# bikuta6/nbody-deep-sim

Hardware: AMD Instinct MI355X
Metric: pair-interactions/sec, direct O(N^2) leapfrog N-body, fp32 (higher is better)
Workload: dtype f32; 1 GPU; Plummer sphere, 65536 particles, direct all-pairs leapfrog step (BASELINE configs[1] shape: 65536 bodies per GPU); n_particles=65536, particles_per_gpu=65536, seed=1234, parallelism=single GPU

## Files before the change

### include/nbd.h

```cpp
#ifndef NBD_H_
#define NBD_H_

#include <stddef.h>
#include <stdint.h>

#ifdef __cplusplus
extern "C" {
#endif

#define NBD_ABI_VERSION 2
#define NBD_E_BADARG (-1)
#define NBD_E_WORKSPACE (-2)
#define NBD_E_UNSUPPORTED (-3)

#define NBD_SRC_PAD 64
#define NBD_CC_TILE 128
#define NBD_CC_GROUPS 8
#define NBD_CC_MAX_RES 4

typedef void* nbd_stream_t;

int nbd_abi_version(void);
size_t nbd_struct_size(const char* name);
const char* nbd_strerror(int code);
// ... 10 lines not shown
int nbd_accel_f32(const float* posm_src, int n_src, const float* posm_tgt, int n_tgt,
                  int tgt_global_offset, float softening_sq, float g_const, float* acc_out,
                  void* workspace, size_t workspace_bytes, nbd_stream_t stream);

size_t nbd_accel_tuned_workspace_bytes(int n_tgt, int slabs);
int nbd_accel_tuned_f32(const float* posm_src, int n_src, int exclude_lo, int exclude_hi, const float* posm_tgt,
                        int n_tgt, int tgt_global_offset, float softening_sq, float g_const, float* acc_out,
                        void* workspace, size_t workspace_bytes, int slabs, int variant, nbd_stream_t stream);

int nbd_shard_plan(int n_total, int lo, int n_local, int* slabs_local, int* chunks_per_wave_local,
                   int* slabs_remote, int* chunks_per_wave_remote);
size_t nbd_shard_workspace_bytes(int n_total, int lo, int n_local);
int nbd_shard_force_local_f32(const float* posm_local, int n_local, float softening_sq, void* workspace,
                              size_t workspace_bytes, int n_total, int lo, nbd_stream_t stream);
int nbd_shard_force_remote_f32(const float* posm_all, int n_total, const float* posm_local, int n_local, int lo,
                               float softening_sq, float g_const, float* acc_out, float* vel, float c_kick,
                               void* workspace, size_t workspace_bytes, nbd_stream_t stream);
int nbd_shard_force_local_uniform_f32(const float* posm_local, int n_local, float softening_sq, void* workspace,
                                      size_t workspace_bytes, int n_total, int lo, nbd_stream_t stream);
int nbd_shard_force_remote_uniform_f32(const float* posm_all, int n_total, const float* posm_local, int n_local, int lo,
                                       float softening_sq, float g_const, float mass_value, float* acc_out, float* vel,
                                       float c_kick, void* workspace, size_t workspace_bytes, nbd_stream_t stream);

int nbd_kick_drift_f32(float* pos, float* vel, const float* acc, const float* mass, int n,
                       float c_kick, float c_drift, float* posm, nbd_stream_t stream);

int nbd_kick_f32(float* vel, const float* acc, int n, float c, nbd_stream_t stream);

int nbd_drift_f32(float* pos, const float* vel, int n, float c, nbd_stream_t stream);

int nbd_snapshot_f32(const float* pos, const float* vel, const float* acc, int n, float* out, nbd_stream_t stream);

size_t nbd_step_workspace_bytes(int n);

size_t nbd_step_workspace_pref_bytes(int n);

int nbd_leapfrog_step_f32(float* pos, float* vel, const float* acc_in, float* acc_out,
                          const float* mass, int n, float dt_half, float dt, float softening_sq,
                          float g_const, float* posm, void* workspace, size_t workspace_bytes,
                          nbd_stream_t stream);

int nbd_leapfrog_step_ev_f32(float* pos, float* vel, const float* acc_in, float* acc_out,
                             const float* mass, int n, float dt_half, float dt, float softening_sq,
                             float g_const, float* posm, void* workspace, size_t workspace_bytes,
                             nbd_stream_t stream, void* ev_force_begin, void* ev_force_end);
int nbd_leapfrog_step_uniform_f32(float* pos, float* vel, const float* acc_in, float* acc_out, const float* mass,
                                  float mass_value, int n, float dt_half, float dt, float softening_sq, float g_const,
                                  float* posm, void* workspace, size_t workspace_bytes, nbd_stream_t stream,
                                  void* ev_force_begin, void* ev_force_end);

size_t nbd_accel_sym_workspace_bytes(int n);
int nbd_accel_sym_uniform_f32(const float* posm, int n, float softening_sq, float g_const, float mass_value,
                              float* acc_out, void* workspace, size_t workspace_bytes, int variant, nbd_stream_t stream);

int nbd_euler_step_f32(float* pos, float* vel, float* acc_out, const float* mass, int n, float dt,
                       float softening_sq, float g_const, float* posm, void* workspace,
                       size_t workspace_bytes, nbd_stream_t stream);

size_t nbd_energy_workspace_bytes(int n);

int nbd_energy_f32(const float* posm, const float* vel, int n, float softening, float g_const,
                   double* out_uk, void* workspace, size_t workspace_bytes, nbd_stream_t stream);

size_t nbd_potential_workspace_bytes(int n_src, int n_tgt);
int nbd_potential_f32(const float* posm_src, int n_src, const float* posm_tgt, int n_tgt, int tgt_global_offset,
                      float softening_sq, float g_const, double* phi_out, void* workspace, size_t workspace_bytes,
                      nbd_stream_t stream);
int nbd_invariants_f64(const float* posm, const float* vel, const double* phi, int n, double* out_row,
                       nbd_stream_t stream);

int nbd_batch_plan(const int* offsets, int n_scenes, int* n_items, int* posm_rows, size_t* plan_bytes,
                   size_t* workspace_bytes);
int nbd_batch_plan_fill(const int* offsets, int n_scenes, void* plan, size_t plan_bytes);
int nbd_batch_pack_posm_f32(const int* offsets, int n_scenes, const void* plan, size_t plan_bytes, const float* pos,
                            const float* mass, float* posm, nbd_stream_t stream);
int nbd_batch_accel_f32(const int* offsets, int n_scenes, const void* plan, size_t plan_bytes, const float* pos,
                        const float* mass, const float* softening_sq, const float* g_const, float* acc_out,
                        float* posm, void* workspace, size_t workspace_bytes, nbd_stream_t stream);
int nbd_batch_leapfrog_step_f32(const int* offsets, int n_scenes, const void* plan, size_t plan_bytes, float* pos,
                                float* vel, const float* acc_in, float* acc_out, const float* mass, const float* dt_half,
                                const float* dt, const float* softening_sq, const float* g_const, float* posm,
                                void* workspace, size_t workspace_bytes, nbd_stream_t stream);
int nbd_batch_euler_step_f32(const int* offsets, int n_scenes, const void* plan, size_t plan_bytes, float* pos,
                             float* vel, float* acc_out, const float* mass, const float* dt, const float* softening_sq,
                             const float* g_const, float* posm, void* workspace, size_t workspace_bytes,
                             nbd_stream_t stream);
int nbd_batch_energies(const int* offsets, int n_scenes, const void* plan, size_t plan_bytes, const float* posm,
                       const float* vel, const float* softening, const float* g_const, double* out_uk, void* workspace,
                       size_t workspace_bytes, nbd_stream_t stream);
int nbd_batch_potential_f32(const int* offsets, int n_scenes, const void* plan, size_t plan_bytes, const float* posm,
                            const float* softening_sq, const float* g_const, double* phi_out, void* workspace,
                            size_t workspace_bytes, nbd_stream_t stream);
int nbd_batch_invariants_f64(const int* offsets, int n_scenes, const void* plan, size_t plan_bytes, const float* posm,
                             const float* vel, const double* phi, double* out_rows, nbd_stream_t stream);

int nbd_batch_hermite_workspace_bytes(const int* offsets, int n_scenes, size_t* bytes);
int nbd_batch_accel_jerk_f32(const int* offsets, int n_scenes, const void* plan, size_t plan_bytes, const float* pos,
                             const float* vel, const float* mass, const float* softening_sq, const float* g_const,
                             float* acc_out, float* jerk_out, float* posm, void* workspace, size_t workspace_bytes,
                             nbd_stream_t stream);
int nbd_batch_hermite_step_f32(const int* offsets, int n_scenes, const void* plan, size_t plan_bytes, float* pos,
                               float* vel, const float* acc_in, const float* jerk_in, float* acc_out, float* jerk_out,
                               const float* mass, const float* hdt, const float* softening_sq, const float* g_const,
                               float* posm, void* workspace, size_t workspace_bytes, nbd_stream_t stream);

size_t nbd_hermite_workspace_bytes(int n);
// ... 398 lines not shown
```

### nbody-deep-sim_amd/csrc/direct_force.hip

```cpp
#include <hip/hip_runtime.h>
#include <string.h>
#include <stdint.h>

#include <type_traits>

#include "../../include/nbd.h"
#include "direct_kernels.h"

namespace {

template <bool MASKED, int KU, bool UNI = false>
__global__ __launch_bounds__(64 * kWaves, KU == 4 ? 8 : 5) void accel_kernel(
    const f4* __restrict__ src, const SrcView sv, const f4* __restrict__ tgt,
    int n_tgt, int tgt_off, float eps2, float scale, float* __restrict__ out, int out_rows, int tile_len) {
  __shared__ f4 lds[kAccelLdsF4];
  const int tz = blockIdx.z * tile_len;
  const int t_base = blockIdx.x * kTgtPerWG;
  accel_body<KU, UNI>(src + tz, sv, std::integral_constant<bool, MASKED>{}, tgt + tz, n_tgt, tgt_off, t_base, blockIdx.y, eps2, scale, lds,
                      out + (size_t)tz * 3 + ((size_t)blockIdx.y * out_rows + t_base) * 3);
}

constexpr int kSymTile = 1024;
constexpr int kSymChunks = kSymTile / kChunk;
constexpr int kSymSlots = 16;
// ... 238 lines not shown
          rz = __builtin_elementwise_fma(-w[u], dz[u], rz);
        }
      }
      rx = f2{rol1(rx.x), rol1(rx.y)};
      ry = f2{rol1(ry.x), rol1(ry.y)};
      rz = f2{rol1(rz.x), rol1(rz.y)};
    }
    float* const mine = react + (j * 8 + wave) * 6 * 64 + lane;
    mine[0 * 64] = rx.x; mine[1 * 64] = rx.y;
    mine[2 * 64] = ry.x; mine[3 * 64] = ry.y;
    mine[4 * 64] = rz.x; mine[5 * 64] = rz.y;
  }
  float* const o_b = out + ((size_t)slot * n + (size_t)tb * kSymTile) * 3;
  float* const o_a = out + ((size_t)slot * n + (size_t)ta * kSymTile) * 3;
  float oldb[6], olda[6];
  if (!init) {
#pragma unroll
    for (int i = 0; i < 6; ++i) oldb[i] = o_b[threadIdx.x + i * 512];
#pragma unroll
    for (int i = 0; i < 6; ++i) olda[i] = o_a[threadIdx.x + i * 512];
  }
  __syncthreads();

#pragma unroll
  for (int i = 0; i < 6; ++i) {
    const int o = threadIdx.x + i * 512;
    const int row = o / 3, comp = o - row * 3;
    const int c = row >> 6, l = row & 63, p = c & (kSym2Pairs - 1), hf = c / kSym2Pairs;
    const float* rs = react + ((p & 1) * 8 + (p >> 1) * 2) * 6 * 64 + (comp * 2 + hf) * 64 + l;
    const float v = rs[0] + rs[6 * 64];
    o_b[o] = init ? v : oldb[i] + v;
  }
  __syncthreads();
#pragma unroll
  for (int t = 0; t < kSym2T; ++t) {
    float* const mo = ldsf + ((sg * 2 + tg) * 3 * kSym2T + t) * 64 + lane;
    mo[0 * kSym2T * 64] = ax[t].x + ax[t].y;
    mo[1 * kSym2T * 64] = ay[t].x + ay[t].y;
    mo[2 * kSym2T * 64] = az[t].x + az[t].y;
  }
  __syncthreads();
#pragma unroll
  for (int i = 0; i < 6; ++i) {
    const int o = threadIdx.x + i * 512;
    const int row = o / 3, comp = o - row * 3;
    const int g = row >> 9, t = (row >> 6) & (kSym2T - 1), l = row & 63;
    const float* os = ldsf + ((g * 3 + comp) * kSym2T + t) * 64 + l;
    constexpr int kSg = 2 * 3 * kSym2T * 64;
    const float v = ((os[0] + os[kSg]) + os[2 * kSg]) + os[3 * kSg];
    o_a[o] = init ? v : olda[i] + v;
  }
}

__global__ __launch_bounds__(256) void finish_kernel(const float* __restrict__ slabs, int n_slabs,
                                                     size_t slab_stride, float g, float* __restrict__ acc,
                                                     float* __restrict__ vel, float c_kick, int n3) {
  __shared__ float part[4][64];
  const int lane = threadIdx.x & 63, w = threadIdx.x >> 6;
  const int i = blockIdx.x * 64 + lane;
  float sum = 0.f;
  if (i < n3)
    for (int s = w; s < n_slabs; s += 4) sum += slabs[s * slab_stride + i];
  part[w][lane] = sum;
  __syncthreads();
  if (w != 0 || i >= n3) return;
  const float a = __fmul_rn(g, (part[0][lane] + part[1][lane]) + (part[2][lane] + part[3][lane]));
  acc[i] = a;
  if (vel) vel[i] = __fadd_rn(vel[i], __fmul_rn(c_kick, a));
}

__global__ __launch_bounds__(256) void pack_kernel(const float* __restrict__ pos,
                                                   const float* __restrict__ mass, int n, int n_pad,
                                                   f4* __restrict__ posm) {
  const int i = blockIdx.x * 256 + threadIdx.x;
  if (i >= n_pad) return;
  f4 v = {0.f, 0.f, 0.f, 0.f};
  if (i < n) v = f4{pos[3 * i], pos[3 * i + 1], pos[3 * i + 2], mass[i]};
  posm[i] = v;
}

__global__ __launch_bounds__(256) void kick_drift_kernel(float* __restrict__ pos, float* __restrict__ vel,
                                                         const float* __restrict__ acc,
                                                         const float* __restrict__ mass, int n, int n_pad,
                                                         float ck, float cd, f4* __restrict__ posm) {
  const int i = blockIdx.x * 256 + threadIdx.x;
  if (i >= n_pad) return;
  f4 pm = {0.f, 0.f, 0.f, 0.f};
  if (i < n) {
    float x[3];
#pragma unroll
    for (int k = 0; k < 3; ++k) {
      float v = vel[3 * i + k];
      if (acc) { v = __fadd_rn(v, __fmul_rn(ck, acc[3 * i + k])); vel[3 * i + k] = v; }
      x[k] = __fadd_rn(pos[3 * i + k], __fmul_rn(cd, v));
      pos[3 * i + k] = x[k];
    }
    pm = f4{x[0], x[1], x[2], mass ? mass[i] : 0.f};
  }
  if (posm) posm[i] = pm;
}

__global__ __launch_bounds__(256) void zero_f32_kernel(float* __restrict__ p, size_t n) {
  const size_t i = (size_t)blockIdx.x * 256 + threadIdx.x;
  if (i < n) p[i] = 0.f;
}

// ... 118 lines not shown
  if (uniform) {
    if (p.variant == 1) { if (masked) NBD_LAUNCH(true, 4, true); else NBD_LAUNCH(false, 4, true); }
    else                { if (masked) NBD_LAUNCH(true, 8, true); else NBD_LAUNCH(false, 8, true); }
  } else {
    if (p.variant == 1) { if (masked) NBD_LAUNCH(true, 4, false); else NBD_LAUNCH(false, 4, false); }
    else                { if (masked) NBD_LAUNCH(true, 8, false); else NBD_LAUNCH(false, 8, false); }
  }
#undef NBD_LAUNCH
  return launch_status();
}

struct SymPlan { int m, core, rem, slots, total_slots; };

SymPlan plan_sym(int n, int slots_avail = 0) {
  SymPlan p;
  p.m = n / kSymTile;
  p.m &= ~1;
  p.core = p.m * kSymTile;
  p.rem = n - p.core;
  const int narrow = p.m < kSymSlots ? p.m : kSymSlots, wide = p.m < kSymSlotsCap ? p.m : kSymSlotsCap;
  const int avail = slots_avail - (p.rem > 0 ? 1 : 0);
  p.slots = avail < narrow ? narrow : (avail < wide ? avail : wide);
  p.total_slots = p.slots + (p.rem > 0 ? 1 : 0);
  return p;
}

size_t sym_workspace_bytes(int n) {
  const SymPlan p = plan_sym(n);
  return p.m < 2 ? 0 : (size_t)p.total_slots * n * 3 * sizeof(float);
}

int sym_slots_avail(int n, size_t workspace_bytes) {
  const size_t s = workspace_bytes / ((size_t)n * 3 * sizeof(float));
  return s > (size_t)kSymSlotsCap + 1 ? kSymSlotsCap + 1 : (int)s;
}

size_t sym_workspace_pref_bytes(int n) {
  const SymPlan p = plan_sym(n);
  if (p.m < 2) return 0;
  const int k = p.m < kSymSlotsPref ? p.m : kSymSlotsPref;
  return (size_t)(k + (p.rem > 0 ? 1 : 0)) * n * 3 * sizeof(float);
}

constexpr int kSymStepMinN = 65536;
bool sym_step(int n, float eps2) { return n >= kSymStepMinN && eps2 >= kEps2Masked; }

int launch_sym(const float* posm, int n, float eps2, float* slots, const SymPlan& sp, hipStream_t st, int variant = 0) {
  const f4* pm = reinterpret_cast<const f4*>(posm);
  const AccelPlan dp = make_plan(kSymTile / kTgtPerWG, 1, kSymChunks);
  int rc = launch_accel(posm, full_view(kSymTile, dp), posm, kSymTile, 0, eps2, 1.0f, slots, dp, st, true, n, sp.m,
                        kSymTile);
  if (rc) return rc;
  const int rounds = sp.m - 1;
  for (int r0 = 0; r0 < rounds;) {
    const int r1 = r0 == 0 ? (sp.slots - 1 < rounds ? sp.slots - 1 : rounds) : (r0 + sp.slots < rounds ? r0 + sp.slots : rounds);
    const int wgs = (r1 - r0) * (sp.m / 2);
    if (variant == 2) accel_sym2_kernel<<<wgs, 512, 0, st>>>(pm, n, sp.m, r0, sp.slots, eps2, slots);
    else if (variant == 1) accel_sym_kernel<2><<<wgs, 512, 0, st>>>(pm, n, sp.m, r0, sp.slots, eps2, slots);
    else accel_sym_kernel<4><<<wgs, 1024, 0, st>>>(pm, n, sp.m, r0, sp.slots, eps2, slots);
    if ((rc = launch_status())) return rc;
    r0 = r1;
  }
  if (sp.rem == 0) return 0;
  const AccelPlan tp = make_plan(ceil_div(sp.rem, kTgtPerWG), sp.total_slots, ceil_div(n, kChunk));
  rc = launch_accel(posm, full_view(n, tp), posm + (size_t)sp.core * 4, sp.rem, sp.core, eps2, 1.0f,
                    slots + (size_t)sp.core * 3, tp, st, true, n);
  if (rc) return rc;
  SrcView sv;
  const AccelPlan cp = make_plan(sp.core / kTgtPerWG, 1, excluded_view(n, 0, sp.core, &sv));
  return launch_accel(posm, sv, posm, sp.core, 0, eps2, 1.0f, slots + (size_t)sp.slots * n * 3, cp, st, true, n);
}

}

extern "C" {

int nbd_abi_version(void) { return NBD_ABI_VERSION; }

size_t nbd_struct_size(const char* name) {
  if (!name) return 0;
#define NBD_SZ(T) if (!strcmp(name, #T)) return sizeof(T);
  NBD_SZ(nbd_gnn_layer_args) NBD_SZ(nbd_gnn_forward_args) NBD_SZ(nbd_knn_pq_args) NBD_SZ(nbd_gnn_train_args)
  NBD_SZ(nbd_gnn_train_grads) NBD_SZ(nbd_cc_train_args) NBD_SZ(nbd_cc_train_grads) NBD_SZ(nbd_cc_pairs_job)
#undef NBD_SZ
  return 0;
}

const char* nbd_strerror(int code) {
  if (code == 0) return "ok";
  if (code == NBD_E_BADARG) return "nbd: bad argument (null/negative/misaligned)";
  if (code == NBD_E_WORKSPACE) return "nbd: workspace too small";
  if (code == NBD_E_UNSUPPORTED) return "nbd: unsupported configuration";
  if (code > 0) return hipGetErrorString((hipError_t)code);
  return "nbd: unknown error";
}

int nbd_posm_padded_len(int n) { return n <= 0 ? 0 : ceil_div(n, kChunk) * kChunk; }

int nbd_pack_posm_f32(const float* pos, const float* mass, int n, float* posm, nbd_stream_t stream) {
  if (n < 0 || (n > 0 && (!pos || !mass || !posm)) || misaligned16(posm)) return NBD_E_BADARG;
  if (n == 0) return 0;
  const int n_pad = nbd_posm_padded_len(n);
  pack_kernel<<<ceil_div(n_pad, 256), 256, 0, (hipStream_t)stream>>>(pos, mass, n, n_pad,
                                                                    reinterpret_cast<f4*>(posm));
  return launch_status();
}

size_t nbd_accel_workspace_bytes(int n_src, int n_tgt) {
  if (n_src <= 0 || n_tgt <= 0) return 0;
  const AccelPlan p = plan_accel(n_src, n_tgt);
  return p.slabs > 1 ? (size_t)p.slabs * n_tgt * 3 * sizeof(float) : 0;
}

int nbd_accel_plan(int n_src, int n_tgt, int* groups, int* slabs, int* chunks_per_wave) {
  if (n_src <= 0 || n_tgt <= 0) return NBD_E_BADARG;
  const AccelPlan p = plan_accel(n_src, n_tgt);
  if (groups) *groups = p.groups;
  if (slabs) *slabs = p.slabs;
  if (chunks_per_wave) *chunks_per_wave = p.cpw;
  return 0;
}

size_t nbd_step_workspace_bytes(int n) {
  if (n <= 0) return 0;
  const size_t all_pairs = (size_t)plan_accel(n, n).slabs * n * 3 * sizeof(float);
  const size_t sym = sym_step(n, kEps2Masked) ? sym_workspace_bytes(n) : 0;
  return sym > all_pairs ? sym : all_pairs;
}

size_t nbd_step_workspace_pref_bytes(int n) {
  if (n <= 0) return 0;
  const size_t least = nbd_step_workspace_bytes(n);
  const size_t pref = sym_step(n, kEps2Masked) ? sym_workspace_pref_bytes(n) : 0;
  return pref > least ? pref : least;
}

size_t nbd_accel_sym_workspace_bytes(int n) { return n <= 0 ? 0 : sym_workspace_bytes(n); }

int nbd_accel_sym_uniform_f32(const float* posm, int n, float softening_sq, float g_const, float mass_value,
                              float* acc_out, void* workspace, size_t workspace_bytes, int variant, nbd_stream_t stream) {
  if (n < 0 || (n > 0 && (!posm || !acc_out)) || misaligned16(posm) || variant < 0 || variant > 2) return NBD_E_BADARG;
  if (n == 0) return 0;
  if (plan_sym(n).m < 2 || softening_sq < kEps2Masked) return NBD_E_UNSUPPORTED;
  if (!workspace || workspace_bytes < sym_workspace_bytes(n)) return NBD_E_WORKSPACE;
  hipStream_t st = (hipStream_t)stream;
  float* slots = static_cast<float*>(workspace);
  const SymPlan sp = plan_sym(n, sym_slots_avail(n, workspace_bytes));
  int rc = launch_sym(posm, n, softening_sq, slots, sp, st, variant);
  if (rc) return rc;
  const int n3 = 3 * n;
  finish_kernel<<<ceil_div(n3, 64), 256, 0, st>>>(slots, sp.total_slots, (size_t)n3, g_const * mass_value,
                                                   acc_out, nullptr, 0.f, n3);
  return launch_status();
}

int nbd_accel_f32(const float* posm_src, int n_src, const float* posm_tgt, int n_tgt,
                  int tgt_global_offset, float softening_sq, float g_const, float* acc_out,
                  void* workspace, size_t workspace_bytes, nbd_stream_t stream) {
  if (n_src < 0 || n_tgt < 0) return NBD_E_BADARG;
  if (n_tgt == 0) return 0;
  if (!acc_out || !posm_tgt || misaligned16(posm_tgt)) return NBD_E_BADARG;
  hipStream_t st = (hipStream_t)stream;
  if (n_src == 0) {
    zero_f32_kernel<<<ceil_div(n_tgt * 3, 256), 256, 0, st>>>(acc_out, (size_t)n_tgt * 3);
    return launch_status();
  }
  if (!posm_src || misaligned16(posm_src)) return NBD_E_BADARG;
  const AccelPlan p = plan_accel(n_src, n_tgt);
  if (p.slabs == 1)
    return launch_accel(posm_src, full_view(n_src, p), posm_tgt, n_tgt, tgt_global_offset, softening_sq,
                        g_const, acc_out, p, st);
  const size_t need = (size_t)p.slabs * n_tgt * 3 * sizeof(float);
  if (!workspace || workspace_bytes < need) return NBD_E_WORKSPACE;
  float* slabs = static_cast<float*>(workspace);
  int rc = launch_accel(posm_src, full_view(n_src, p), posm_tgt, n_tgt, tgt_global_offset, softening_sq,
                        1.0f, slabs, p, st);
  if (rc) return rc;
  const int n3 = n_tgt * 3;
  finish_kernel<<<ceil_div(n3, 64), 256, 0, st>>>(slabs, p.slabs, (size_t)n3, g_const, acc_out,
                                                   nullptr, 0.f, n3);
  return launch_status();
}

size_t nbd_accel_tuned_workspace_bytes(int n_tgt, int slabs) {
  if (n_tgt <= 0 || slabs <= 0) return 0;
  return (size_t)slabs * n_tgt * 3 * sizeof(float);
}

int nbd_accel_tuned_f32(const float* posm_src, int n_src, int exclude_lo, int exclude_hi, const float* posm_tgt,
                        int n_tgt, int tgt_global_offset, float softening_sq, float g_const, float* acc_out,
                        void* workspace, size_t workspace_bytes, int slabs, int variant, nbd_stream_t stream) {
  if (n_src <= 0 || n_tgt <= 0 || slabs < 1 || slabs > kMaxSlabs || variant < 0 || variant > 1) return NBD_E_BADARG;
  if (exclude_lo < 0 || exclude_hi < exclude_lo || exclude_hi > n_src) return NBD_E_BADARG;
  if (!acc_out || !posm_tgt || !posm_src || misaligned16(posm_tgt) || misaligned16(posm_src)) return NBD_E_BADARG;
  if (!workspace || workspace_bytes < nbd_accel_tuned_workspace_bytes(n_tgt, slabs)) return NBD_E_WORKSPACE;
  hipStream_t st = (hipStream_t)stream;
  SrcView sv;
  const AccelPlan p =
      make_plan(ceil_div(n_tgt, kTgtPerWG), slabs, excluded_view(n_src, exclude_lo, exclude_hi, &sv), variant);
  float* sl = static_cast<float*>(workspace);
  const int n3 = n_tgt * 3;
// ... 105 lines not shown
  return shard_force_remote(posm_all, n_total, posm_local, n_local, lo, softening_sq, g_const * mass_value, acc_out, vel,
                            c_kick, workspace, workspace_bytes, stream, true);
}

int nbd_kick_drift_f32(float* pos, float* vel, const float* acc, const float* mass, int n,
                       float c_kick, float c_drift, float* posm, nbd_stream_t stream) {
  if (n < 0 || (n > 0 && (!pos || !vel)) || (posm && (!mass || misaligned16(posm)))) return NBD_E_BADARG;
  if (n == 0) return 0;
  const int n_pad = posm ? nbd_posm_padded_len(n) : n;
  kick_drift_kernel<<<ceil_div(n_pad, 256), 256, 0, (hipStream_t)stream>>>(
      pos, vel, acc, mass, n, n_pad, c_kick, c_drift, reinterpret_cast<f4*>(posm));
  return launch_status();
}

int nbd_kick_f32(float* vel, const float* acc, int n, float c, nbd_stream_t stream) {
  if (n < 0 || (n > 0 && (!vel || !acc))) return NBD_E_BADARG;
  if (n == 0) return 0;
  axpy_kernel<<<ceil_div(3 * n, 256), 256, 0, (hipStream_t)stream>>>(vel, acc, c, 3 * n);
  return launch_status();
}

int nbd_drift_f32(float* pos, const float* vel, int n, float c, nbd_stream_t stream) {
  if (n < 0 || (n > 0 && (!pos || !vel))) return NBD_E_BADARG;
  if (n == 0) return 0;
  axpy_kernel<<<ceil_div(3 * n, 256), 256, 0, (hipStream_t)stream>>>(pos, vel, c, 3 * n);
  return launch_status();
}

int nbd_snapshot_f32(const float* pos, const float* vel, const float* acc, int n, float* out, nbd_stream_t stream) {
  if (n < 0 || (n > 0 && (!pos || !vel || !acc || !out))) return NBD_E_BADARG;
  if (n == 0) return 0;
  snapshot_kernel<<<ceil_div(3 * n, 256), 256, 0, (hipStream_t)stream>>>(pos, vel, acc, 3 * n, out);
  return launch_status();
}

static int step_force(float* pos, float* vel, const float* acc_in, float* acc_out, const float* mass, int n, bool euler,
                      float c_kick, float c_drift, float softening_sq, float g_scale, bool uniform, float* posm,
                      void* workspace, size_t workspace_bytes, nbd_stream_t stream, void* ev_force_begin,
                      void* ev_force_end) {
  if (n < 0) return NBD_E_BADARG;
  if (n == 0) return 0;
  if (!pos || !vel || (!euler && !acc_in) || !acc_out || !mass || !posm || misaligned16(posm)) return NBD_E_BADARG;
  hipStream_t st = (hipStream_t)stream;
  const bool sym = uniform && sym_step(n, softening_sq);
  const AccelPlan p = plan_accel(n, n);
  const size_t need = sym ? sym_workspace_bytes(n) : (size_t)p.slabs * n * 3 * sizeof(float);
  if (!workspace || workspace_bytes < need) return NBD_E_WORKSPACE;
  int rc = euler ? nbd_pack_posm_f32(pos, mass, n, posm, stream)
                 : nbd_kick_drift_f32(pos, vel, acc_in, mass, n, c_kick, c_drift, posm, stream);
  if (rc) return rc;
  float* slabs = static_cast<float*>(workspace);
  if (ev_force_begin && (rc = check(hipEventRecord((hipEvent_t)ev_force_begin, st)))) return rc;
  const SymPlan sp = plan_sym(n, sym ? sym_slots_avail(n, workspace_bytes) : 0);
  if (sym) rc = launch_sym(posm, n, softening_sq, slabs, sp, st, 2);
  else rc = launch_accel(posm, full_view(n, p), posm, n, 0, softening_sq, 1.0f, slabs, p, st, uniform);
  if (rc) return rc;
  if (ev_force_end && (rc = check(hipEventRecord((hipEvent_t)ev_force_end, st)))) return rc;
  const int n3 = 3 * n;
  const int n_slabs = sym ? sp.total_slots : p.slabs;
  finish_kernel<<<ceil_div(n3, 64), 256, 0, st>>>(slabs, n_slabs, (size_t)n3, g_scale, acc_out, vel, c_kick, n3);
  return launch_status();
}

int nbd_leapfrog_step_ev_f32(float* pos, float* vel, const float* acc_in, float* acc_out,
                          const float* mass, int n, float dt_half, float dt, float softening_sq,
                          float g_const, float* posm, void* workspace, size_t workspace_bytes,
                          nbd_stream_t stream, void* ev_force_begin, void* ev_force_end) {
  return step_force(pos, vel, acc_in, acc_out, mass, n, false, dt_half, dt, softening_sq, g_const, false, posm,
                    workspace, workspace_bytes, stream, ev_force_begin, ev_force_end);
}

int nbd_leapfrog_step_uniform_f32(float* pos, float* vel, const float* acc_in, float* acc_out, const float* mass,
                                  float mass_value, int n, float dt_half, float dt, float softening_sq, float g_const,
                                  float* posm, void* workspace, size_t workspace_bytes, nbd_stream_t stream,
                                  void* ev_force_begin, void* ev_force_end) {
  return step_force(pos, vel, acc_in, acc_out, mass, n, false, dt_half, dt, softening_sq, g_const * mass_value, true,
                    posm, workspace, workspace_bytes, stream, ev_force_begin, ev_force_end);
}

int nbd_leapfrog_step_f32(float* pos, float* vel, const float* acc_in, float* acc_out,
                          const float* mass, int n, float dt_half, float dt, float softening_sq,
                          float g_const, float* posm, void* workspace, size_t workspace_bytes,
                          nbd_stream_t stream) {
  return nbd_leapfrog_step_ev_f32(pos, vel, acc_in, acc_out, mass, n, dt_half, dt, softening_sq, g_const,
                                  posm, workspace, workspace_bytes, stream, nullptr, nullptr);
}

int nbd_euler_step_f32(float* pos, float* vel, float* acc_out, const float* mass, int n, float dt,
                       float softening_sq, float g_const, float* posm, void* workspace,
                       size_t workspace_bytes, nbd_stream_t stream) {
  const int rc = step_force(pos, vel, nullptr, acc_out, mass, n, true, dt, 0.f, softening_sq, g_const, false, posm,
                            workspace, workspace_bytes, stream, nullptr, nullptr);
  if (rc) return rc;
  return nbd_drift_f32(pos, vel, n, dt, stream);
}

size_t nbd_energy_workspace_bytes(int n) {
  if (n <= 0) return 0;
  const int groups = ceil_div(n, kTgtPerWG);
  return ((size_t)groups * energy_slabs(groups) + (size_t)ceil_div(n, 256)) * sizeof(double);
}

int nbd_energy_f32(const float* posm, const float* vel, int n, float softening, float g_const,
                   double* out_uk, void* workspace, size_t workspace_bytes, nbd_stream_t stream) {
  if (n < 0 || !out_uk) return NBD_E_BADARG;
  hipStream_t st = (hipStream_t)stream;
  if (n == 0) {
// ... 22 lines not shown
```

### nbody-deep-sim_amd/nbd/_lib.py

```python
from __future__ import annotations

import ctypes
import os
import subprocess
from ctypes import c_char_p, c_double, c_float, c_int, c_int64, c_size_t, c_void_p, POINTER

import torch

_HERE = os.path.dirname(os.path.abspath(__file__))
CSRC_DIR = os.path.normpath(os.path.join(_HERE, "..", "csrc"))
LIB_PATH = os.environ.get("NBD_LIB_OVERRIDE") or os.path.join(CSRC_DIR, "libnbd_hip.so")


class NbdError(RuntimeError):
    pass


class NbdUnsupported(NbdError):
    """A configuration a fast path does not cover (NBD_E_UNSUPPORTED, or the Python-side check in front of it): callers that
    probe a path catch THIS and fall back; any other NbdError is a real failure and propagates."""


def build(verbose: bool = False) -> str:
    res = subprocess.run(["make", "-C", CSRC_DIR, "-j4"], capture_output=True, text=True)
# ... 72 lines not shown
                ("ln_g", c_void_p), ("ln_b", c_void_p), ("head_w", _PF), ("head_b", _PF)]


class CcPairsJob(ctypes.Structure):
    _fields_ = [("rowptr", c_void_p), ("centres", c_void_p), ("deg", c_void_p), ("edge_capacity", c_int64),
                ("filter_resolution", c_int), ("cell_map", c_void_p), ("n_cells", c_int), ("adjoint", c_int),
                ("pair_lists", c_void_p), ("pair_lists_bytes", c_size_t)]


CC_MAX_RES = 4
ABI_VERSION = 2

_F = POINTER(c_float)
SIGNATURES = {
    "nbd_abi_version": (c_int, []),
    "nbd_strerror": (c_char_p, [c_int]),
    "nbd_posm_padded_len": (c_int, [c_int]),
    "nbd_pack_posm_f32": (c_int, [c_void_p, c_void_p, c_int, c_void_p, c_void_p]),
    "nbd_accel_workspace_bytes": (c_size_t, [c_int, c_int]),
    "nbd_accel_plan": (c_int, [c_int, c_int, POINTER(c_int), POINTER(c_int), POINTER(c_int)]),
    "nbd_accel_f32": (c_int, [c_void_p, c_int, c_void_p, c_int, c_int, c_float, c_float, c_void_p,
                              c_void_p, c_size_t, c_void_p]),
    "nbd_accel_tuned_workspace_bytes": (c_size_t, [c_int, c_int]),
    "nbd_accel_tuned_f32": (c_int, [c_void_p, c_int, c_int, c_int, c_void_p, c_int, c_int, c_float, c_float,
                                    c_void_p, c_void_p, c_size_t, c_int, c_int, c_void_p]),
    "nbd_shard_plan": (c_int, [c_int, c_int, c_int, POINTER(c_int), POINTER(c_int), POINTER(c_int),
                               POINTER(c_int)]),
    "nbd_shard_workspace_bytes": (c_size_t, [c_int, c_int, c_int]),
    "nbd_shard_force_local_f32": (c_int, [c_void_p, c_int, c_float, c_void_p, c_size_t, c_int, c_int, c_void_p]),
    "nbd_shard_force_remote_f32": (c_int, [c_void_p, c_int, c_void_p, c_int, c_int, c_float, c_float, c_void_p,
                                           c_void_p, c_float, c_void_p, c_size_t, c_void_p]),
    "nbd_shard_force_local_uniform_f32": (c_int, [c_void_p, c_int, c_float, c_void_p, c_size_t, c_int, c_int, c_void_p]),
    "nbd_shard_force_remote_uniform_f32": (c_int, [c_void_p, c_int, c_void_p, c_int, c_int, c_float, c_float, c_float,
                                                   c_void_p, c_void_p, c_float, c_void_p, c_size_t, c_void_p]),
    "nbd_kick_drift_f32": (c_int, [c_void_p, c_void_p, c_void_p, c_void_p, c_int, c_float, c_float,
                                   c_void_p, c_void_p]),
    "nbd_kick_f32": (c_int, [c_void_p, c_void_p, c_int, c_float, c_void_p]),
    "nbd_drift_f32": (c_int, [c_void_p, c_void_p, c_int, c_float, c_void_p]),
    "nbd_snapshot_f32": (c_int, [c_void_p, c_void_p, c_void_p, c_int, c_void_p, c_void_p]),
    "nbd_step_workspace_bytes": (c_size_t, [c_int]),
    "nbd_step_workspace_pref_bytes": (c_size_t, [c_int]),
    "nbd_leapfrog_step_f32": (c_int, [c_void_p, c_void_p, c_void_p, c_void_p, c_void_p, c_int,
                                      c_float, c_float, c_float, c_float, c_void_p, c_void_p,
                                      c_size_t, c_void_p]),
    "nbd_leapfrog_step_ev_f32": (c_int, [c_void_p, c_void_p, c_void_p, c_void_p, c_void_p, c_int,
                                         c_float, c_float, c_float, c_float, c_void_p, c_void_p,
                                         c_size_t, c_void_p, c_void_p, c_void_p]),
    "nbd_leapfrog_step_uniform_f32": (c_int, [c_void_p, c_void_p, c_void_p, c_void_p, c_void_p, c_float, c_int,
                                              c_float, c_float, c_float, c_float, c_void_p, c_void_p,
                                              c_size_t, c_void_p, c_void_p, c_void_p]),
    "nbd_accel_sym_workspace_bytes": (c_size_t, [c_int]),
    "nbd_accel_sym_uniform_f32": (c_int, [c_void_p, c_int, c_float, c_float, c_float, c_void_p, c_void_p, c_size_t,
                                          c_int, c_void_p]),
    "nbd_euler_step_f32": (c_int, [c_void_p, c_void_p, c_void_p, c_void_p, c_int, c_float, c_float,
                                   c_float, c_void_p, c_void_p, c_size_t, c_void_p]),
    "nbd_energy_workspace_bytes": (c_size_t, [c_int]),
    "nbd_energy_f32": (c_int, [c_void_p, c_void_p, c_int, c_float, c_float, c_void_p, c_void_p,
                               c_size_t, c_void_p]),
    "nbd_potential_workspace_bytes": (c_size_t, [c_int, c_int]),
    "nbd_potential_f32": (c_int, [c_void_p, c_int, c_void_p, c_int, c_int, c_float, c_float, c_void_p, c_void_p,
                                  c_size_t, c_void_p]),
    "nbd_invariants_f64": (c_int, [c_void_p, c_void_p, c_void_p, c_int, c_void_p, c_void_p]),
    "nbd_batch_potential_f32": (c_int, [c_void_p, c_int, c_void_p, c_size_t, c_void_p, c_void_p, c_void_p, c_void_p,
                                        c_void_p, c_size_t, c_void_p]),
    "nbd_batch_invariants_f64": (c_int, [c_void_p, c_int, c_void_p, c_size_t, c_void_p, c_void_p, c_void_p, c_void_p,
                                         c_void_p]),
    "nbd_batch_plan": (c_int, [c_void_p, c_int, POINTER(c_int), POINTER(c_int), POINTER(c_size_t), POINTER(c_size_t)]),
    "nbd_batch_plan_fill": (c_int, [c_void_p, c_int, c_void_p, c_size_t]),
    "nbd_batch_pack_posm_f32": (c_int, [c_void_p, c_int, c_void_p, c_size_t, c_void_p, c_void_p, c_void_p, c_void_p]),
    "nbd_batch_accel_f32": (c_int, [c_void_p, c_int, c_void_p, c_size_t, c_void_p, c_void_p, c_void_p, c_void_p,
                                    c_void_p, c_void_p, c_void_p, c_size_t, c_void_p]),
    "nbd_batch_leapfrog_step_f32": (c_int, [c_void_p, c_int, c_void_p, c_size_t, c_void_p, c_void_p, c_void_p, c_void_p,
                                            c_void_p, c_void_p, c_void_p, c_void_p, c_void_p, c_void_p, c_void_p, c_size_t,
                                            c_void_p]),
    "nbd_batch_euler_step_f32": (c_int, [c_void_p, c_int, c_void_p, c_size_t, c_void_p, c_void_p, c_void_p, c_void_p,
                                         c_void_p, c_void_p, c_void_p, c_void_p, c_void_p, c_size_t, c_void_p]),
    "nbd_batch_energies": (c_int, [c_void_p, c_int, c_void_p, c_size_t, c_void_p, c_void_p, c_void_p, c_void_p, c_void_p,
                                   c_void_p, c_size_t, c_void_p]),
    "nbd_batch_hermite_workspace_bytes": (c_int, [c_void_p, c_int, POINTER(c_size_t)]),
    "nbd_batch_accel_jerk_f32": (c_int, [c_void_p, c_int, c_void_p, c_size_t, c_void_p, c_void_p, c_void_p, c_void_p,
                                         c_void_p, c_void_p, c_void_p, c_void_p, c_void_p, c_size_t, c_void_p]),
    "nbd_batch_hermite_step_f32": (c_int, [c_void_p, c_int, c_void_p, c_size_t, c_void_p, c_void_p, c_void_p, c_void_p,
                                           c_void_p, c_void_p, c_void_p, c_void_p, c_void_p, c_void_p, c_void_p, c_void_p,
                                           c_size_t, c_void_p]),
    "nbd_hermite_workspace_bytes": (c_size_t, [c_int]),
    "nbd_hermite_pack_f32": (c_int, [c_void_p, c_void_p, c_void_p, c_void_p, c_void_p, c_int, c_double, c_void_p,
                                     c_void_p, c_void_p]),
    "nbd_accel_jerk_f32": (c_int, [c_void_p, c_void_p, c_int, c_float, c_float, c_void_p, c_void_p, c_void_p, c_size_t,
                                   c_int, c_void_p]),
    "nbd_hermite_step_f32": (c_int, [c_void_p, c_void_p, c_void_p, c_void_p, c_void_p, c_void_p, c_void_p, c_int,
                                     c_double, c_float, c_float, c_void_p, c_void_p, c_size_t, c_void_p]),
    "nbd_hermite_shard_plan": (c_int, [c_int, c_int, c_int, POINTER(c_int), POINTER(c_int), POINTER(c_int),
                                       POINTER(c_int)]),
    "nbd_hermite_shard_workspace_bytes": (c_size_t, [c_int, c_int, c_int]),
    "nbd_hermite_shard_predict_f32": (c_int, [c_void_p, c_void_p, c_void_p, c_void_p, c_void_p, c_int, c_double,
                                              c_void_p, c_int, c_void_p]),
    "nbd_hermite_shard_force_local_f32": (c_int, [c_void_p, c_int, c_float, c_void_p, c_size_t, c_int, c_int, c_void_p]),
    "nbd_hermite_shard_force_remote_f32": (c_int, [c_void_p, c_int, c_void_p, c_int, c_int, c_float, c_float, c_void_p,
                                                   c_void_p, c_void_p, c_void_p, c_void_p, c_void_p, c_double, c_void_p,
                                                   c_size_t, c_void_p]),
    "nbd_hermite_f64_workspace_bytes": (c_size_t, [c_int]),
    "nbd_hermite_f64_plan": (c_int, [c_int, POINTER(c_int), POINTER(c_int), POINTER(c_int)]),
    "nbd_hermite_f64_pack": (c_int, [c_void_p, c_void_p, c_void_p, c_void_p, c_void_p, c_int, c_double, c_void_p,
                                     c_void_p, c_void_p]),
    "nbd_accel_jerk_f64": (c_int, [c_void_p, c_void_p, c_int, c_double, c_double, c_void_p, c_void_p, c_void_p, c_size_t,
                                   c_int, c_void_p]),
# ... 238 lines not shown
```

### nbody-deep-sim_amd/nbd/direct.py

```python
from __future__ import annotations

import ctypes
import os

import numpy as np
import torch

from . import _lib


def _chk(t: torch.Tensor, shape, name: str, dtype=torch.float32):
    if not isinstance(t, torch.Tensor) or not t.is_cuda:
        raise _lib.NbdError(f"{name}: expected a CUDA/HIP tensor (no CPU fallback on this path)")
    if t.dtype != dtype or not t.is_contiguous():
        raise _lib.NbdError(f"{name}: expected contiguous {dtype}, got {t.dtype} contiguous={t.is_contiguous()}")
    if shape is not None and tuple(t.shape) != tuple(shape):
        raise _lib.NbdError(f"{name}: expected shape {tuple(shape)}, got {tuple(t.shape)}")


def padded_len(n: int) -> int:
    return _lib.lib().nbd_posm_padded_len(int(n))


def _chk_packed(dtype, pos_rows, vel_rows, n: int):
# ... 124 lines not shown

def _nbytes(t: torch.Tensor) -> int:
    return t.numel() * t.element_size()


def step_workspace(n: int, device) -> torch.Tensor:
    L = _lib.lib()
    least, pref = L.nbd_step_workspace_bytes(n), L.nbd_step_workspace_pref_bytes(n)
    cap = os.environ.get("NBD_SYM_SLOTS")
    if cap is not None and pref > least:
        pref = min(pref, (max(int(cap), 0) + (1 if n % 2048 else 0)) * n * 12)
    return alloc_bytes(max(least, pref), device)


def kick_drift(pos, vel, acc, mass, c_kick: float, c_drift: float, posm=None) -> None:
    n = pos.shape[0]
    _chk(pos, (n, 3), "pos"); _chk(vel, (n, 3), "vel")
    if acc is not None:
        _chk(acc, (n, 3), "acc")
    if posm is not None:
        _chk(mass, (n,), "mass")
        if posm.dtype != torch.float32 or not posm.is_contiguous() or posm.shape[0] < padded_len(n):
            raise _lib.NbdError("posm: need contiguous fp32 (>= padded_len(n), 4)")
    with _lib.on_device(pos.device):
        _lib.check(_lib.lib().nbd_kick_drift_f32(pos.data_ptr(), vel.data_ptr(), _lib.ptr(acc),
                                                 _lib.ptr(mass), n, c_kick, c_drift, _lib.ptr(posm),
                                                 _lib.current_stream(pos.device)), "nbd_kick_drift_f32")


def kick(vel, acc, c: float) -> None:
    n = vel.shape[0]
    _chk(vel, (n, 3), "vel"); _chk(acc, (n, 3), "acc")
    with _lib.on_device(vel.device):
        _lib.check(_lib.lib().nbd_kick_f32(vel.data_ptr(), acc.data_ptr(), n, c,
                                           _lib.current_stream(vel.device)), "nbd_kick_f32")


def drift(pos, vel, c: float) -> None:
    n = pos.shape[0]
    _chk(pos, (n, 3), "pos"); _chk(vel, (n, 3), "vel")
    with _lib.on_device(pos.device):
        _lib.check(_lib.lib().nbd_drift_f32(pos.data_ptr(), vel.data_ptr(), n, c,
                                            _lib.current_stream(pos.device)), "nbd_drift_f32")


def snapshot(pos, vel, acc, out) -> None:
    n = pos.shape[0]
    _chk(pos, (n, 3), "pos"); _chk(vel, (n, 3), "vel"); _chk(acc, (n, 3), "acc"); _chk(out, (3, n, 3), "out")
    with _lib.on_device(pos.device):
        _lib.check(_lib.lib().nbd_snapshot_f32(pos.data_ptr(), vel.data_ptr(), acc.data_ptr(), n, out.data_ptr(),
                                               _lib.current_stream(pos.device)), "nbd_snapshot_f32")


def uniform_mass(mass: torch.Tensor):
    if mass.numel() == 0:
        return None
    lo, hi = torch.aminmax(mass)
    lo, hi = float(lo), float(hi)
    return lo if (lo == hi and lo > 0.0 and lo != float("inf")) else None


def leapfrog_step(pos, vel, acc_in, acc_out, mass, dt_half: float, dt: float, softening_sq: float,
                  g_const: float, posm, workspace, ev_begin=None, ev_end=None, uniform=None) -> None:
    n = pos.shape[0]
    for t, nm in ((pos, "pos"), (vel, "vel"), (acc_in, "acc_in"), (acc_out, "acc_out")):
        _chk(t, (n, 3), nm)
    _chk(mass, (n,), "mass"); _chk(posm, (padded_len(n), 4), "posm")
    with _lib.on_device(pos.device):
        if uniform is not None:
            _lib.check(_lib.lib().nbd_leapfrog_step_uniform_f32(
                pos.data_ptr(), vel.data_ptr(), acc_in.data_ptr(), acc_out.data_ptr(), mass.data_ptr(), float(uniform), n,
                dt_half, dt, softening_sq, g_const, posm.data_ptr(), workspace.data_ptr(), _nbytes(workspace),
                _lib.current_stream(pos.device),
                None if ev_begin is None else ev_begin.cuda_event,
                None if ev_end is None else ev_end.cuda_event), "nbd_leapfrog_step_uniform_f32")
            return
        _lib.check(_lib.lib().nbd_leapfrog_step_ev_f32(
            pos.data_ptr(), vel.data_ptr(), acc_in.data_ptr(), acc_out.data_ptr(), mass.data_ptr(), n,
            dt_half, dt, softening_sq, g_const, posm.data_ptr(), workspace.data_ptr(), _nbytes(workspace),
            _lib.current_stream(pos.device),
            None if ev_begin is None else ev_begin.cuda_event,
            None if ev_end is None else ev_end.cuda_event), "nbd_leapfrog_step_f32")


def euler_step(pos, vel, acc_out, mass, dt: float, softening_sq: float, g_const: float, posm,
               workspace) -> None:
    n = pos.shape[0]
    for t, nm in ((pos, "pos"), (vel, "vel"), (acc_out, "acc_out")):
        _chk(t, (n, 3), nm)
    _chk(mass, (n,), "mass"); _chk(posm, (padded_len(n), 4), "posm")
    with _lib.on_device(pos.device):
        _lib.check(_lib.lib().nbd_euler_step_f32(
            pos.data_ptr(), vel.data_ptr(), acc_out.data_ptr(), mass.data_ptr(), n, dt, softening_sq,
            g_const, posm.data_ptr(), workspace.data_ptr(), _nbytes(workspace),
            _lib.current_stream(pos.device)), "nbd_euler_step_f32")


def energy(posm, vel, n: int, softening: float, g_const: float, out_uk=None, workspace=None):
    _chk(posm, (padded_len(n), 4), "posm"); _chk(vel, (n, 3), "vel")
    dev = vel.device
    if out_uk is None:
        out_uk = torch.empty(2, dtype=torch.float64, device=dev)
    _chk(out_uk, (2,), "out_uk", torch.float64)
    need = _lib.lib().nbd_energy_workspace_bytes(n)
    if workspace is None or _nbytes(workspace) < need:
        workspace = alloc_bytes(need, dev)
# ... 685 lines not shown
```

Before: 6902 billion pair-interactions/s.

## Add single-launch symmetric tile-pair force kernel with LDS reaction reduction

```diff
diff --git a/include/nbd.h b/include/nbd.h
--- a/include/nbd.h
+++ b/include/nbd.h
@@ -86,6 +86,8 @@
 size_t nbd_accel_sym_workspace_bytes(int n);
 int nbd_accel_sym_uniform_f32(const float* posm, int n, float softening_sq, float g_const, float mass_value,
                               float* acc_out, void* workspace, size_t workspace_bytes, int variant, nbd_stream_t stream);
+int nbd_accel_sym3_uniform_f32(const float* posm, int n, float softening_sq, float g_const, float mass_value,
+                               float* acc_out, void* workspace, size_t workspace_bytes, nbd_stream_t stream);
 
 int nbd_euler_step_f32(float* pos, float* vel, float* acc_out, const float* mass, int n, float dt,
                        float softening_sq, float g_const, float* posm, void* workspace,
diff --git a/nbody-deep-sim_amd/csrc/direct_force.hip b/nbody-deep-sim_amd/csrc/direct_force.hip
--- a/nbody-deep-sim_amd/csrc/direct_force.hip
+++ b/nbody-deep-sim_amd/csrc/direct_force.hip
@@ -314,6 +314,143 @@
   }
 }
 
+constexpr int kSym3Steps = 4;
+
+__device__ __forceinline__ void sym3_step(const f2 sx, const f2 sy, const f2 sz, f2 (&txy)[kSym2T], f2 (&tzz)[kSym2T / 2],
+                                          const f2 e2, f2 (&ax)[kSym2T], f2 (&ay)[kSym2T], f2 (&az)[kSym2T], f2& rx,
+                                          f2& ry, f2& rz) {
+#pragma unroll
+  for (int t = 0; t < kSym2T; ++t) asm volatile("" : "+v"(txy[t]));
+#pragma unroll
+  for (int t = 0; t < kSym2T / 2; ++t) asm volatile("" : "+v"(tzz[t]));
+#pragma unroll
+  for (int g = 0; g < kSym2T; g += kSym2G) {
+    f2 dx[kSym2G], dy[kSym2G], dz[kSym2G], s[kSym2G], w[kSym2G];
+#pragma unroll
+    for (int u = 0; u < kSym2G; ++u) {
+      const int t = g + u;
+      const float tz = (t & 1) ? tzz[t >> 1].y : tzz[t >> 1].x;
+      dx[u] = sx - f2{txy[t].x, txy[t].x}; dy[u] = sy - f2{txy[t].y, txy[t].y}; dz[u] = sz - f2{tz, tz};
+    }
+    __builtin_amdgcn_sched_barrier(0);
+#pragma unroll
+    for (int u = 0; u < kSym2G; ++u) s[u] = __builtin_elementwise_fma(dx[u], dx[u], e2);
+    __builtin_amdgcn_sched_barrier(0);
+#pragma unroll
+    for (int u = 0; u < kSym2G; ++u) s[u] = __builtin_elementwise_fma(dy[u], dy[u], s[u]);
+    __builtin_amdgcn_sched_barrier(0);
+#pragma unroll
+    for (int u = 0; u < kSym2G; ++u) s[u] = __builtin_elementwise_fma(dz[u], dz[u], s[u]);
+    __builtin_amdgcn_sched_barrier(0);
+#pragma unroll
+    for (int u = 0; u < kSym2G; ++u) s[u] = f2{__builtin_amdgcn_rsqf(s[u].x), __builtin_amdgcn_rsqf(s[u].y)};
+    __builtin_amdgcn_sched_barrier(0);
+#pragma unroll
+    for (int u = 0; u < kSym2G; ++u) w[u] = s[u] * s[u];
+    __builtin_amdgcn_sched_barrier(0);
+#pragma unroll
+    for (int u = 0; u < kSym2G; ++u) w[u] = w[u] * s[u];
+    __builtin_amdgcn_sched_barrier(0);
+#pragma unroll
+    for (int u = 0; u < kSym2G; ++u) {
+      const int t = g + u;
+      ax[t] = __builtin_elementwise_fma(w[u], dx[u], ax[t]);
+      ay[t] = __builtin_elementwise_fma(w[u], dy[u], ay[t]);
+      az[t] = __builtin_elementwise_fma(w[u], dz[u], az[t]);
+      rx = __builtin_elementwise_fma(-w[u], dx[u], rx);
+      ry = __builtin_elementwise_fma(-w[u], dy[u], ry);
+      rz = __builtin_elementwise_fma(-w[u], dz[u], rz);
+    }
+  }
+  rx = f2{rol1(rx.x), rol1(rx.y)};
+  ry = f2{rol1(ry.x), rol1(ry.y)};
+  rz = f2{rol1(rz.x), rol1(rz.y)};
+}
+
+__global__ __launch_bounds__(512, 4) void accel_sym3_kernel(const f4* __restrict__ posm, int n, int m, float eps2,
+                                                            float* __restrict__ out) {
+  constexpr int kPairF2 = 3 * 128;
+  constexpr int kImgF = kSym2Pairs * kPairF2 * 2;
+  constexpr int kTileF = kSymTile * 3;
+  constexpr int kReactF = 2 * kTileF;
+  constexpr int kOwnF = 4 * kTileF;
+  static_assert(kImgF + kReactF == kOwnF, "one 48-KiB LDS image");
+  __shared__ f4 lds[kOwnF / 4];
+  float* const ldsf = reinterpret_cast<float*>(lds);
+  f2* const img = reinterpret_cast<f2*>(lds);
+  float* const react = ldsf + kImgF;
+
+  int ta, tb, slot;
+  bool init;
+  sym_round_match(blockIdx.x, m, 0, m, ta, tb, slot, init);
+
+  const int lane = threadIdx.x & 63;
+  const int wave = __builtin_amdgcn_readfirstlane(threadIdx.x >> 6);
+  const int tg = wave & 1, sg = wave >> 1;
+  {
+    const f4 u = posm[tb * kSymTile + wave * kChunk + lane];
+    const f4 v = posm[tb * kSymTile + (wave + kSym2Pairs) * kChunk + lane];
+    f2* const e = img + wave * kPairF2 + lane;
+    e[0] = e[64] = f2{u.x, v.x};
+    e[128] = e[192] = f2{u.y, v.y};
+    e[256] = e[320] = f2{u.z, v.z};
+  }
+  const int row0 = ta * kSymTile + tg * 512 + lane;
+  f2 txy[kSym2T], tzz[kSym2T / 2];
+  f2 ax[kSym2T], ay[kSym2T], az[kSym2T];
+#pragma unroll
+  for (int t = 0; t < kSym2T; ++t) {
+    const f4 q = posm[row0 + t * 64];
+    txy[t] = f2{q.x, q.y};
+    if (t & 1) tzz[t >> 1].y = q.z; else tzz[t >> 1].x = q.z;
+    ax[t] = ay[t] = az[t] = f2{0.f, 0.f};
+  }
+  f2 e2 = {eps2, eps2};
+  asm volatile("" : "+v"(e2));
+  __syncthreads();
+
+#pragma unroll 1
+  for (int j = 0; j < 2; ++j) {
+    const int p = sg * 2 + j;
+    const f2* const b = img + p * kPairF2 + lane;
+    f2 rx = {0.f, 0.f}, ry = {0.f, 0.f}, rz = {0.f, 0.f};
+#pragma unroll 1
+    for (int k = 0; k < kChunk; k += kSym3Steps) {
+#pragma unroll
+      for (int u = 0; u < kSym3Steps; ++u)
+        sym3_step(b[k + u], b[128 + k + u], b[256 + k + u], txy, tzz, e2, ax, ay, az, rx, ry, rz);
+    }
+    float* const mine = react + tg * kTileF + (p * kChunk + lane) * 3;
+    mine[0] = rx.x; mine[1] = ry.x; mine[2] = rz.x;
+    mine[kSym2Pairs * kChunk * 3 + 0] = rx.y; mine[kSym2Pairs * kChunk * 3 + 1] = ry.y; mine[kSym2Pairs * kChunk * 3 + 2] = rz.y;
+  }
+  float* const o_b = out + ((size_t)slot * n + (size_t)tb * kSymTile) * 3;
+  float* const o_a = out + ((size_t)slot * n + (size_t)ta * kSymTile) * 3;
+  __syncthreads();
+
+#pragma unroll
+  for (int i = 0; i < 6; ++i) {
+    const int o = threadIdx.x + i * 512;
+    o_b[o] = react[o] + react[kTileF + o];
+  }
+  __syncthreads();
+  {
+    float* const mo = ldsf + sg * kTileF + (tg * 512 + lane) * 3;
+#pragma unroll
+    for (int t = 0; t < kSym2T; ++t) {
+      mo[t * 64 * 3 + 0] = ax[t].x + ax[t].y;
+      mo[t * 64 * 3 + 1] = ay[t].x + ay[t].y;
+      mo[t * 64 * 3 + 2] = az[t].x + az[t].y;
+    }
+  }
+  __syncthreads();
+#pragma unroll
+  for (int i = 0; i < 6; ++i) {
+    const int o = threadIdx.x + i * 512;
+    o_a[o] = ((ldsf[o] + ldsf[kTileF + o]) + ldsf[2 * kTileF + o]) + ldsf[3 * kTileF + o];
+  }
+}
+
 __global__ __launch_bounds__(256) void finish_kernel(const float* __restrict__ slabs, int n_slabs,
                                                      size_t slab_stride, float g, float* __restrict__ acc,
                                                      float* __restrict__ vel, float c_kick, int n3) {
@@ -538,7 +675,12 @@
                         kSymTile);
   if (rc) return rc;
   const int rounds = sp.m - 1;
-  for (int r0 = 0; r0 < rounds;) {
+  if (variant == 3 && sp.slots != sp.m) variant = 2;
+  if (variant == 3) {
+    accel_sym3_kernel<<<rounds * (sp.m / 2), 512, 0, st>>>(pm, n, sp.m, eps2, slots);
+    if ((rc = launch_status())) return rc;
+  }
+  for (int r0 = variant == 3 ? rounds : 0; r0 < rounds;) {
     const int r1 = r0 == 0 ? (sp.slots - 1 < rounds ? sp.slots - 1 : rounds) : (r0 + sp.slots < rounds ? r0 + sp.slots : rounds);
     const int wgs = (r1 - r0) * (sp.m / 2);
     if (variant == 2) accel_sym2_kernel<<<wgs, 512, 0, st>>>(pm, n, sp.m, r0, sp.slots, eps2, slots);
@@ -633,6 +775,24 @@
   float* slots = static_cast<float*>(workspace);
   const SymPlan sp = plan_sym(n, sym_slots_avail(n, workspace_bytes));
   int rc = launch_sym(posm, n, softening_sq, slots, sp, st, variant);
+  if (rc) return rc;
+  const int n3 = 3 * n;
+  finish_kernel<<<ceil_div(n3, 64), 256, 0, st>>>(slots, sp.total_slots, (size_t)n3, g_const * mass_value,
+                                                   acc_out, nullptr, 0.f, n3);
+  return launch_status();
+}
+
+int nbd_accel_sym3_uniform_f32(const float* posm, int n, float softening_sq, float g_const, float mass_value,
+                               float* acc_out, void* workspace, size_t workspace_bytes, nbd_stream_t stream) {
+  if (n < 0 || (n > 0 && (!posm || !acc_out)) || misaligned16(posm)) return NBD_E_BADARG;
+  if (n == 0) return 0;
+  if (plan_sym(n).m < 2 || softening_sq < kEps2Masked) return NBD_E_UNSUPPORTED;
+  if (!workspace || workspace_bytes < sym_workspace_bytes(n)) return NBD_E_WORKSPACE;
+  const SymPlan sp = plan_sym(n, sym_slots_avail(n, workspace_bytes));
+  if (sp.slots != sp.m) return NBD_E_UNSUPPORTED;
+  hipStream_t st = (hipStream_t)stream;
+  float* slots = static_cast<float*>(workspace);
+  int rc = launch_sym(posm, n, softening_sq, slots, sp, st, 3);
   if (rc) return rc;
   const int n3 = 3 * n;
   finish_kernel<<<ceil_div(n3, 64), 256, 0, st>>>(slots, sp.total_slots, (size_t)n3, g_const * mass_value,
@@ -844,7 +1004,7 @@
   float* slabs = static_cast<float*>(workspace);
   if (ev_force_begin && (rc = check(hipEventRecord((hipEvent_t)ev_force_begin, st)))) return rc;
   const SymPlan sp = plan_sym(n, sym ? sym_slots_avail(n, workspace_bytes) : 0);
-  if (sym) rc = launch_sym(posm, n, softening_sq, slabs, sp, st, 2);
+  if (sym) rc = launch_sym(posm, n, softening_sq, slabs, sp, st, 3);
   else rc = launch_accel(posm, full_view(n, p), posm, n, 0, softening_sq, 1.0f, slabs, p, st, uniform);
   if (rc) return rc;
   if (ev_force_end && (rc = check(hipEventRecord((hipEvent_t)ev_force_end, st)))) return rc;
diff --git a/nbody-deep-sim_amd/nbd/_lib.py b/nbody-deep-sim_amd/nbd/_lib.py
--- a/nbody-deep-sim_amd/nbd/_lib.py
+++ b/nbody-deep-sim_amd/nbd/_lib.py
@@ -148,6 +148,8 @@
     "nbd_accel_sym_workspace_bytes": (c_size_t, [c_int]),
     "nbd_accel_sym_uniform_f32": (c_int, [c_void_p, c_int, c_float, c_float, c_float, c_void_p, c_void_p, c_size_t,
                                           c_int, c_void_p]),
+    "nbd_accel_sym3_uniform_f32": (c_int, [c_void_p, c_int, c_float, c_float, c_float, c_void_p, c_void_p, c_size_t,
+                                           c_void_p]),
     "nbd_euler_step_f32": (c_int, [c_void_p, c_void_p, c_void_p, c_void_p, c_int, c_float, c_float,
                                    c_float, c_void_p, c_void_p, c_size_t, c_void_p]),
     "nbd_energy_workspace_bytes": (c_size_t, [c_int]),
diff --git a/nbody-deep-sim_amd/nbd/direct.py b/nbody-deep-sim_amd/nbd/direct.py
--- a/nbody-deep-sim_amd/nbd/direct.py
+++ b/nbody-deep-sim_amd/nbd/direct.py
@@ -200,6 +200,19 @@
                                                _lib.current_stream(pos.device)), "nbd_snapshot_f32")
 
 
+def accel_sym3(posm: torch.Tensor, n: int, softening_sq: float, g_const: float, mass_value: float,
+               workspace: torch.Tensor, out: torch.Tensor | None = None) -> torch.Tensor:
+    _chk(posm, (padded_len(n), 4), "posm")
+    if out is None:
+        out = torch.empty((n, 3), dtype=torch.float32, device=posm.device)
+    _chk(out, (n, 3), "acc_out")
+    with _lib.on_device(posm.device):
+        _lib.check(_lib.lib().nbd_accel_sym3_uniform_f32(
+            posm.data_ptr(), n, float(softening_sq), float(g_const), float(mass_value), out.data_ptr(),
+            workspace.data_ptr(), _nbytes(workspace), _lib.current_stream(posm.device)), "nbd_accel_sym3_uniform_f32")
+    return out
+
+
 def uniform_mass(mass: torch.Tensor):
     if mass.numel() == 0:
         return None
```

Result: no change. 6960 billion pair-interactions/s (median of 6 runs) (+0.8%).
